# PolarisRisingWar/rgb-experiment

Hardware: AMD Instinct MI355X
Metric: aggregated edges/sec (full-graph GCN d=128, reference epoch = train fwd+bwd+Adam + 2 eval fwd) (higher is better)
Workload: dtype f32

## Files before the change

include/rgbx_hip.h:

```cpp
#ifndef RGBX_HIP_H
#define RGBX_HIP_H

#include <stddef.h>
#include <stdint.h>

#ifdef __cplusplus
extern "C" {
#endif

#define RGBX_VERSION 501

#define RGBX_OK 0
#define RGBX_E_ARG (-1)
#define RGBX_E_RANGE (-2)
#define RGBX_E_ALIGN (-3)
#define RGBX_E_WS (-4)
#define RGBX_E_SHAPE (-5)

typedef void* rgbx_stream_t;

enum {
  RGBX_LOOPS_KEEP = 0,
  RGBX_LOOPS_ADD_REMAINING = 1,
  RGBX_LOOPS_REMOVE_ADD = 2
// ... 307 lines not shown
int rgbx_gatv2_bwd_src_f32(const int32_t* rowptr_t, const int32_t* col_t, const int32_t* t2f, const float* xl,
                           int64_t ldl, const float* xr, int64_t ldr, const float* att, const float* nodeq,
                           const float* gout, int64_t ldg, float* g_xl, int64_t ldgl, int64_t N, int H, int C,
                           float slope, const uint32_t* seed, float p_drop, const rgbx_row_split_t* split,
                           rgbx_stream_t stream);

int rgbx_gatv2_draws_u8(const uint32_t* seed, int64_t nnz, int H, float p_drop, uint8_t* keep, rgbx_stream_t stream);


int rgbx_gemm_tn_workspace_bytes(int64_t K, int64_t M, int64_t N, size_t* bytes);

int rgbx_gemm_tn_f32(const float* A, int64_t lda, const float* B, int64_t ldb, float* C, int64_t ldc,
                     float* a_colsum, int64_t K, int64_t M, int64_t N, float alpha, void* workspace,
                     size_t workspace_bytes, rgbx_stream_t stream);


int rgbx_bn_scratch_doubles(int64_t N, int64_t d, int64_t* count);

int rgbx_bn_stats_f32(const float* x, int64_t ldx, int64_t N, int64_t d, double* sums, double* scratch,
                      int64_t scratch_doubles, rgbx_stream_t stream);

int rgbx_bn_finalize_f32(const double* packed, const float* weight, const float* bias, float eps, float momentum,
                         float* running_mean, float* running_var, float* mean, float* rstd, float* scale,
                         float* shift, int64_t d, rgbx_stream_t stream);

int rgbx_fold_bn_linear_f32(const float* W, int64_t ldw, const float* Wr, int64_t ldwr, const float* bias,
                            const float* bias2, const float* gamma, const float* beta, const float* running_mean,
                            const float* running_var, float eps, float* wt, float* wrt, float* b_out, int64_t Nout,
                            int64_t K, rgbx_stream_t stream);

// ... 92 lines not shown
```

rgb_experiment_amd/_lib.py:

```python
import ctypes
import os

import torch

_HERE = os.path.dirname(os.path.abspath(__file__))
LIB_PATH = os.path.join(_HERE, "csrc", "librgbx_hip.so")

_P = ctypes.c_void_p
_I64 = ctypes.c_int64
_I = ctypes.c_int
_F = ctypes.c_float

class RowSplit(ctypes.Structure):
    _fields_ = [("threshold", ctypes.c_int32), ("n_chunks", ctypes.c_int32), ("n_long", ctypes.c_int32),
                ("chunk_begin", ctypes.c_void_p), ("chunk_end", ctypes.c_void_p), ("chunk_row", ctypes.c_void_p),
                ("long_row", ctypes.c_void_p),
                ("long_chunk_ptr", ctypes.c_void_p), ("partial", ctypes.c_void_p)]


class MultiOut(ctypes.Structure):
    _fields_ = [(f, t) for name in ("sum", "mean", "var", "std", "max", "argmax", "min", "argmin")
                for f, t in ((name, ctypes.c_void_p), ("ld_" + name, ctypes.c_int64))]


# ... 83 lines not shown
                                  _P, _P],
    "rgbx_supergat_sample_negatives": [_P, _I64, _I64, _P, _I64, _I, _P, _P, _P],
    "rgbx_supergat_neg_loss_fwd_f32": [_P, _I64, _P, _P, _I64, _I, _I, _P, _I64, _P, _P],
    "rgbx_supergat_neg_loss_bwd_f32": [_P, _I64, _P, _P, _I64, _I, _I, _P, _P, _I64, _P],
    "rgbx_supergat_draws_u8": [_P, _I64, _I, _F, _F, _P, _P, _P],
    "rgbx_gatv2_supported": [_I, _I],
    "rgbx_gatv2_fwd_f32": [_P, _P, _P, _I64, _P, _I64, _P, _P, _P, _I64, _P, _P, _I64, _I, _I, _F, _P, _F, _P, _P],
    "rgbx_gatv2_att_partial_floats": [_I64, _I, _I, _P, ctypes.POINTER(ctypes.c_int64)],
    "rgbx_gatv2_bwd_dst_f32": [_P, _P, _P, _I64, _P, _I64, _P, _P, _P, _P, _I64, _P, _P, _I64, _P, _P, _I64, _P, _P, _I64,
                               _I64, _I, _I, _F, _P, _F, _P, _P],
    "rgbx_gatv2_bwd_src_f32": [_P, _P, _P, _P, _I64, _P, _I64, _P, _P, _P, _I64, _P, _I64, _I64, _I, _I, _F, _P, _F, _P,
                               _P],
    "rgbx_gatv2_draws_u8": [_P, _I64, _I, _F, _P, _P],
    "rgbx_gemm_tn_workspace_bytes": [_I64, _I64, _I64, ctypes.POINTER(ctypes.c_size_t)],
    "rgbx_gemm_tn_f32": [_P, _I64, _P, _I64, _P, _I64, _P, _I64, _I64, _I64, _F, _P, ctypes.c_size_t, _P],
    "rgbx_bn_scratch_doubles": [_I64, _I64, ctypes.POINTER(ctypes.c_int64)],
    "rgbx_bn_stats_f32": [_P, _I64, _I64, _I64, _P, _P, _I64, _P],
    "rgbx_bn_finalize_f32": [_P, _P, _P, _F, _F, _P, _P, _P, _P, _P, _P, _I64, _P],
    "rgbx_fold_bn_linear_f32": [_P, _I64, _P, _I64, _P, _P, _P, _P, _P, _P, _F, _P, _P, _P, _I64, _I64, _P],
    "rgbx_bn_bwd_finalize_f32": [_P, _P, _P, _P, _P, _P, _P, _P, _P, _P, _I64, _P],
    "rgbx_affine_cols_f32": [_P, _I64, _P, _P, _P, _I64, _I64, _I64, _P],
    "rgbx_bn_bwd_reduce_f32": [_P, _I64, _P, _I64, _P, _P, _I64, _I64, _P, _P, _I64, _P],
    "rgbx_bn_bwd_apply_f32": [_P, _I64, _P, _I64, _P, _P, _P, _P, _P, _P, _I64, _I64, _I64, _P],
    "rgbx_masked_nll_scratch_doubles": [_I64, _I, ctypes.POINTER(ctypes.c_int64)],
    "rgbx_masked_nll_fwd_f32": [_P, _I64, _P, _P, _I64, _I64, _P, _P, _I64, _I, _P],
    "rgbx_masked_ce_fwd_f32": [_P, _I64, _P, _P, _I64, _I64, _P, _P, _I64, _P],
    "rgbx_masked_ce_fwd_blocked_f32": [_P, _I64, _I64, _P, _P, _P, _I64, _I64, _P, _P, _I64, _P],
    "rgbx_masked_ce_bwd_f32": [_P, _I64, _P, _P, _I64, _I64, _P, _P, _I64, _P],
    "rgbx_masked_nll_bwd_f32": [_P, _P, _I64, _I64, _P, _P, _I64, _P],
    "rgbx_coalesce_workspace_bytes": [_I64, _I64, _I, ctypes.POINTER(ctypes.c_size_t)],
# ... 38 lines not shown
    if _lib is not None:
        return _lib
    if not os.path.exists(LIB_PATH):
        raise RuntimeError(
            f"rgb_experiment_amd: {LIB_PATH} is not built — run `python -c 'import __graft_entry__ as g; "
            "g.build()'` (or `make -C rgb_experiment_amd/csrc`). There is no CPU fallback.")
    _lib = bind(LIB_PATH)
    return _lib


def use(lib):
    global _lib
    _lib = lib


def check(rc, what):
    if rc != 0:
        msg = load().rgbx_last_error_string().decode(errors="replace")
        kind = "argument error" if rc < 0 else "hipError"
        raise RuntimeError(f"{what} failed ({kind} {rc}): {msg}")


def require_device(*tensors):
    for t in tensors:
        if t is not None and not t.is_cuda:
            raise RuntimeError(
                "rgb_experiment_amd: the message-passing path runs in HIP kernels on an MI355X device; "
                f"got a tensor on '{t.device}'. There is no CPU fallback (oracle/ is test-only).")


# ... 16 lines not shown
```

rgb_experiment_amd/csrc/bn.hip:

```cpp
#include "rgbx_common.h"

namespace rgbx {
namespace {

constexpr int kMaxBlocks = 1024;

struct ColMap {
  int cv;
  int rg;
};

__host__ __device__ inline ColMap col_map(int d, int vec) {
  int cv = (d + vec - 1) / vec;
  if (cv > 256) cv = 256;
  ColMap m{cv, 256 / cv};
  return m;
}

template <int VEC, bool BWD>
__global__ void __launch_bounds__(256)
col_reduce_kernel(const float* __restrict__ a, int64_t lda, const float* __restrict__ b, int64_t ldb,
                  const float* __restrict__ mean, const float* __restrict__ rstd, int64_t N, int d,
                  double* __restrict__ part) {
  extern __shared__ double sh[];
// ... 109 lines not shown
  const int per_row = (d + VEC - 1) / VEC;
  const int64_t total = N * per_row;
  for (int64_t idx = (int64_t)blockIdx.x * blockDim.x + threadIdx.x; idx < total;
       idx += (int64_t)gridDim.x * blockDim.x) {
    const int64_t r = idx / per_row;
    const int c = (int)(idx % per_row) * VEC;
    float g[VEC], v[VEC], mu[VEC], rs[VEC], a[VEC], b[VEC], k[VEC];
    load_vec<VEC>(g, gy + r * ldg + c);
    load_vec<VEC>(v, x + r * ldx + c);
    load_vec<VEC>(mu, mean + c);
    load_vec<VEC>(rs, rstd + c);
    load_vec<VEC>(a, ca + c);
    load_vec<VEC>(b, cb + c);
    load_vec<VEC>(k, ck + c);
#pragma unroll
    for (int i = 0; i < VEC; ++i) g[i] = (g[i] - a[i] - (v[i] - mu[i]) * rs[i] * b[i]) * k[i];
    store_vec<VEC>(gx + r * ldgx + c, g);
  }
}

int reduce_grid(int64_t N, int d, int vec) {
  const ColMap M = col_map(d, vec);
  int64_t b = cdiv(N, (int64_t)M.rg * 16);
  if (b > kMaxBlocks) b = kMaxBlocks;
  return (int)(b < 1 ? 1 : b);
}

bool vec4_ok(int64_t d, std::initializer_list<const void*> ptrs, std::initializer_list<int64_t> lds) {
  bool ok = d % 4 == 0;
  for (const void* p : ptrs) ok = ok && aligned16(p);
  for (int64_t ld : lds) ok = ok && ld % 4 == 0;
// ... 218 lines not shown
```

rgb_experiment_amd/csrc/gemm.hip:

```cpp
#include "rgbx_common.h"

namespace rgbx {
namespace {

constexpr int BM = 128, BN = 128, KT = 32;
using f32x16 = __attribute__((ext_vector_type(16))) float;

template <int W>
__device__ __forceinline__ void stage_tile(float* __restrict__ lds, const float* __restrict__ src,
                                           int64_t ld, int64_t k0, int64_t k_end, int c0, int ncols) {
  const int tid = threadIdx.x;
#pragma unroll 4
  for (int p = 0; p < KT * W / 256; ++p) {
    const int idx = p * 256 + tid;
    const int r = idx / W, c = idx % W;
    const int64_t k = k0 + r;
    lds[r * W + c] = (k < k_end && c0 + c < ncols) ? src[k * ld + c0 + c] : 0.f;
  }
}

template <int W>
__device__ __forceinline__ void fetch_tile(float4 (&regs)[KT * (W / 4) / 256], const float* __restrict__ src, int64_t ld,
                                           int64_t k0, int64_t k_end, int c0, int ncols) {
#pragma unroll
// ... 4 lines not shown
    regs[p] = make_float4(0.f, 0.f, 0.f, 0.f);
    if (k < k_end && c0 + c < ncols) regs[p] = *reinterpret_cast<const float4*>(src + k * ld + c0 + c);
  }
}

template <int W>
__device__ __forceinline__ void put_tile(float* __restrict__ lds, const float4 (&regs)[KT * (W / 4) / 256]) {
#pragma unroll
  for (int p = 0; p < KT * (W / 4) / 256; ++p) {
    const int idx = p * 256 + threadIdx.x;
    const int r = idx / (W / 4), c = (idx % (W / 4)) * 4;
    *reinterpret_cast<float4*>(lds + r * W + c) = regs[p];
  }
}

template <bool VEC4, int MT>
__global__ void __launch_bounds__(256)
gemm_tn_partial_kernel(const float* __restrict__ A, int64_t lda, const float* __restrict__ B, int64_t ldb,
                       float* __restrict__ part, float* __restrict__ colpart, int64_t K, int M, int N,
                       int64_t slab) {
  constexpr int MI = MT / 64;
  __shared__ float lds[KT * (MT + 128)];
  float* la = lds;
  float* lb = lds + KT * MT;
  const int split = blockIdx.x;
  const int m0 = blockIdx.y * MT, n0 = blockIdx.z * BN;
  const int64_t k_begin = (int64_t)split * slab;
  const int64_t k_end = k_begin + slab < K ? k_begin + slab : K;
  const int wave = threadIdx.x >> 6, lane = threadIdx.x & 63;
  const int wm = (wave >> 1) * (MT / 2), wn = (wave & 1) * 64;
  const int kr = lane >> 5, cc = lane & 31;

  f32x16 acc[MI][2];
#pragma unroll
  for (int i = 0; i < MI; ++i)
#pragma unroll
    for (int j = 0; j < 2; ++j)
#pragma unroll
      for (int r = 0; r < 16; ++r) acc[i][j][r] = 0.f;
// ... 7 lines not shown
    }
#pragma unroll 4
    for (int kk = 0; kk < KT; kk += 2) {
      float a[MI];
#pragma unroll
      for (int i = 0; i < MI; ++i) a[i] = la[(kk + kr) * MT + wm + i * 32 + cc];
      const float b0 = lb[(kk + kr) * 128 + wn + cc];
      const float b1 = lb[(kk + kr) * 128 + wn + 32 + cc];
#pragma unroll
      for (int i = 0; i < MI; ++i) {
        acc[i][0] = __builtin_amdgcn_mfma_f32_32x32x2f32(a[i], b0, acc[i][0], 0, 0, 0);
        acc[i][1] = __builtin_amdgcn_mfma_f32_32x32x2f32(a[i], b1, acc[i][1], 0, 0, 0);
      }
    }
  };
  if constexpr (VEC4) {
    float4 ra[KT * (MT / 4) / 256], rb[KT * 32 / 256];
    fetch_tile<MT>(ra, A, lda, k_begin, k_end, m0, M);
    fetch_tile<128>(rb, B, ldb, k_begin, k_end, n0, N);
    for (int64_t k0 = k_begin; k0 < k_end; k0 += KT) {
      __syncthreads();
      put_tile<MT>(la, ra);
      put_tile<128>(lb, rb);
      __syncthreads();
      if (k0 + KT < k_end) {
        fetch_tile<MT>(ra, A, lda, k0 + KT, k_end, m0, M);
        fetch_tile<128>(rb, B, ldb, k0 + KT, k_end, n0, N);
      }
      consume();
    }
  } else {
// ... 53 lines not shown
  return (int)s;
}

}
}

using namespace rgbx;

extern "C" int rgbx_gemm_tn_workspace_bytes(int64_t K, int64_t M, int64_t N, size_t* bytes) {
  if (!bytes || K < 0 || M < 0 || N < 0) return fail(RGBX_E_ARG, "gemm_tn_workspace_bytes: bad argument");
  if (M >= INT32_MAX || N >= INT32_MAX) return fail(RGBX_E_RANGE, "gemm_tn: M or N exceeds int32");
  *bytes = (size_t)choose_splits(K, (int)M, (int)N) * ((size_t)M * (size_t)N + (size_t)M) * sizeof(float);
  return RGBX_OK;
}

extern "C" int rgbx_gemm_tn_f32(const float* A, int64_t lda, const float* B, int64_t ldb, float* C,
                                int64_t ldc, float* a_colsum, int64_t K, int64_t M, int64_t N, float alpha,
                                void* workspace, size_t workspace_bytes, rgbx_stream_t stream) {
  if (K < 0 || M < 0 || N < 0) return fail(RGBX_E_ARG, "gemm_tn: negative size");
  if (M == 0 || N == 0) return RGBX_OK;
  if (!C || (K > 0 && (!A || !B))) return fail(RGBX_E_ARG, "gemm_tn: null pointer");
  if (M >= INT32_MAX || N >= INT32_MAX) return fail(RGBX_E_RANGE, "gemm_tn: M or N exceeds int32");
  if (lda < M || ldb < N || ldc < N) return fail(RGBX_E_ARG, "gemm_tn: leading dimension too small");
  size_t need = 0;
  if (int rc = rgbx_gemm_tn_workspace_bytes(K, M, N, &need)) return rc;
  if (!workspace || workspace_bytes < need)
    return fail(RGBX_E_WS, "gemm_tn: workspace %zu < %zu bytes", workspace_bytes, need);
  hipStream_t s = (hipStream_t)stream;
  const int S = choose_splits(K, (int)M, (int)N);
  const int64_t slab = cdiv(cdiv(K > 0 ? K : 1, S), KT) * KT;
  float* part = static_cast<float*>(workspace);
  float* colpart = a_colsum ? part + (size_t)S * M * N : nullptr;
  const int mt = tile_rows((int)M);
  dim3 grid(S, (unsigned)cdiv(M, mt), (unsigned)cdiv(N, BN));
  const bool v4 = aligned16(A) && aligned16(B) && lda % 4 == 0 && ldb % 4 == 0;
#define RGBX_GEMM_TN(V4, MT) \
  gemm_tn_partial_kernel<V4, MT><<<grid, 256, 0, s>>>(A, lda, B, ldb, part, colpart, K, (int)M, (int)N, slab)
  if (v4) { if (mt == 64) RGBX_GEMM_TN(true, 64); else RGBX_GEMM_TN(true, 128); }
  else { if (mt == 64) RGBX_GEMM_TN(false, 64); else RGBX_GEMM_TN(false, 128); }
#undef RGBX_GEMM_TN
  RGBX_CHECK_LAUNCH("gemm_tn_partial_kernel");
  const int64_t MN = M * N;
  int64_t rb = cdiv(MN, 32);
  if (rb > kMaxGrid) rb = kMaxGrid;
  gemm_tn_reduce_kernel<<<(int)rb, 256, 0, s>>>(part, S, MN, C, (int)N, ldc, alpha);
  RGBX_CHECK_LAUNCH("gemm_tn_reduce_kernel");
  if (a_colsum) {
    gemm_tn_reduce_kernel<<<(int)cdiv(M, 32), 256, 0, s>>>(colpart, S, M, a_colsum, (int)M, M, 1.0f);
    RGBX_CHECK_LAUNCH("gemm_tn_reduce_kernel");
  }
  return RGBX_OK;
}
```

rgb_experiment_amd/csrc/rgbx_common.h:

```cpp
#pragma once
#include <cstring>
#include <hip/hip_runtime.h>

#include <algorithm>
#include <cstdarg>
#include <cstdint>
#include <cstdio>
#include <initializer_list>

#include "../../include/rgbx_hip.h"

namespace rgbx {

constexpr int kWave = 64;

char* err_buf();

inline int fail(int code, const char* fmt, ...) {
  va_list ap;
  va_start(ap, fmt);
  vsnprintf(err_buf(), 256, fmt, ap);
  va_end(ap);
  return code;
}
// ... 31 lines not shown
  if constexpr (VEC == 4) { v[0] = t.x; v[1] = t.y; v[2] = t.z; v[3] = t.w; }
  else if constexpr (VEC == 2) { v[0] = t.x; v[1] = t.y; }
  else { v[0] = t; }
}

template <int VEC>
__device__ __forceinline__ void store_vec(float* p, const float (&v)[VEC]) {
  using V = typename VecT<VEC>::type;
  V t;
  if constexpr (VEC == 4) { t.x = v[0]; t.y = v[1]; t.z = v[2]; t.w = v[3]; }
  else if constexpr (VEC == 2) { t.x = v[0]; t.y = v[1]; }
  else { t = v[0]; }
  *reinterpret_cast<V*>(p) = t;
}

constexpr int kMaxGrid = 256 * 8 * 4;

}
```

rgb_experiment_amd/models/_stack.py:

```python
import torch
import torch.nn as nn
import torch.nn.functional as F

from ..nn import BatchNorm1d


class ModelOutput(dict):

    _LAZY = ("out", "x")

    def __init__(self, logits):
        super().__init__(emb=logits)

    def _log_probs(self):
        out = F.log_softmax(dict.__getitem__(self, "emb"), dim=1)
        dict.__setitem__(self, "out", out)
        dict.__setitem__(self, "x", out)
        return out

    def __missing__(self, key):
        if key in self._LAZY:
            return self._log_probs()
        raise KeyError(key)

# ... 95 lines not shown
                res = conv.forward_folded(x, edge_index, folded[i], ce=ce if i == last else None, **ew)
                if res is not None:
                    x = res
                    continue
            extra = dict(ew)
            if (bn is not None and bn.training and torch.is_grad_enabled() and getattr(conv, "emits_colsums", False)
                    and hasattr(bn, "begin_training_step")):
                extra["want_colsums"] = True
            if (i == last and ce is not None and getattr(conv, "accepts_ce", False)
                    and (not isinstance(ce[1], (tuple, list)) or getattr(conv, "accepts_ce_pair", False))):
                extra["ce"] = ce
            if pending is not None:
                sums = getattr(x, ops.COLSUMS, None)
                after = getattr(conv, "forward_after_bn", None)
                if after is not None:
                    x, pending = after(x, edge_index, pending, colsums=sums, **extra), bn
                    continue
                x, pending = (pending(x, colsums=sums) if sums is not None else pending(x)), None
            affine = None
            if bn is not None and getattr(conv, "folds_post_affine", False) and not torch.is_grad_enabled():
                fold = getattr(bn, "eval_affine", None)
                affine = fold() if fold is not None else None
            if affine is not None:
                x = conv(x, edge_index, post_affine=affine, **ew)
            else:
                x, pending = conv(x, edge_index, **extra), bn
        if ce is not None and not isinstance(x, tuple):
            x = ops.ce_from_logits(x, ce[0], ce[1])
        return x


# ... 152 lines not shown
```

rgb_experiment_amd/nn/batchnorm.py:

```python
import ctypes

import torch
import torch.nn as nn

from .. import _lib


def _scratch(n, d, device):
    cnt = ctypes.c_int64(0)
    _lib.check(_lib.load().rgbx_bn_scratch_doubles(n, d, ctypes.byref(cnt)), "rgbx_bn_scratch_doubles")
    return torch.empty(cnt.value, dtype=torch.float64, device=device), cnt.value


def column_sums(x):
    if not x.is_cuda:
        xd = x.double()
        return torch.stack([xd.sum(0), (xd * xd).sum(0)])
    px, ldx = _lib.mat(x, "x")
    n, d = x.shape
    sums = torch.empty((2, d), dtype=torch.float64, device=x.device)
    scratch, cnt = _scratch(n, d, x.device)
    _lib.check(_lib.load().rgbx_bn_stats_f32(px, ldx, n, d, _lib.ptr(sums), _lib.ptr(scratch), cnt, _lib.stream_ptr()),
               "rgbx_bn_stats_f32")
    return sums
# ... 75 lines not shown
    else:
        mean64 = packed[:d] / n
        var64 = (packed[d:2 * d] / n - mean64 * mean64).clamp_(min=0.0)
        mean, var = mean64.float(), var64.float()
        rstd = torch.rsqrt(var + eps)
        scale = weight.detach() * rstd
        shift = bias.detach() - mean * scale
        if running is not None:
            rm, rv, mom = running
            unbiased = var * (n / (n - 1).clamp(min=1)).float()
            rm.mul_(1 - mom).add_(mean, alpha=mom)
            rv.mul_(1 - mom).add_(unbiased, alpha=mom)
    return mean, rstd, scale, shift, n


def train_backward(gy, x, weight, mean, rstd, n, reduce, grads_out=None, sums=None):
    gy = gy if gy.stride(-1) == 1 else gy.contiguous()
    d = x.size(1)
    if sums is None:
        local = bwd_sums(gy, x, mean, rstd)
        glob = reduce(local.reshape(-1).clone())
    else:
        local, glob = sums
    if gy.is_cuda:
        ca, cb, ck = (torch.empty(d, dtype=torch.float32, device=gy.device) for _ in range(3))
        gw, gb = grads_out if grads_out is not None else (torch.empty(d, dtype=torch.float32, device=gy.device)
                                                          for _ in range(2))
        _lib.check(_lib.load().rgbx_bn_bwd_finalize_f32(
            _lib.ptr(glob), _lib.ptr(local), _lib.ptr(n), _lib.ptr(weight.detach().contiguous()), _lib.ptr(rstd),
            _lib.ptr(ca), _lib.ptr(cb), _lib.ptr(ck), _lib.ptr(gw), _lib.ptr(gb), d, _lib.stream_ptr()),
            "rgbx_bn_bwd_finalize_f32")
    else:
        glob = glob.reshape(2, -1)
        ca = (glob[0] / n).float().contiguous()
        cb = (glob[1] / n).float().contiguous()
        ck = (weight * rstd).contiguous()
        gw, gb = local[1].float(), local[0].float()
        if grads_out is not None:
            grads_out[0].copy_(gw)
            grads_out[1].copy_(gb)
            gw, gb = grads_out
    return bwd_apply(gy, x, mean, rstd, ca, cb, ck), gw, gb


class _AffineCols(torch.autograd.Function):

    @staticmethod
    def forward(ctx, x, scale, shift):
        x = x if x.stride(-1) == 1 else x.contiguous()
        ctx.save_for_backward(x, scale)
        return affine_cols(x, scale.detach().contiguous(), shift.detach().contiguous())

    @staticmethod
    def backward(ctx, gy):
        x, scale = ctx.saved_tensors
        gy = gy if gy.stride(-1) == 1 else gy.contiguous()
# ... 47 lines not shown
```

rgb_experiment_amd/ops.py:

```python
import ctypes

import torch

from . import _lib

_EVENT_SINK = None


def set_event_sink(sink):
    global _EVENT_SINK
    _EVENT_SINK = sink


class Kind(str):
    variant = None


class _Timed:
    def __init__(self, kind, variant=None):
        if variant is not None and _EVENT_SINK is not None:
            kind = Kind(kind)
            kind.variant = variant
        self.kind = kind

# ... 848 lines not shown
    def forward(ctx, z, weight, bias, root_weight, x_root, want_colsums):
        out, _, cs = fused_layer(z, weight_t(weight), bias=None if bias is None else bias.detach(),
                                 x_root=x_root if root_weight is not None else None,
                                 wt_root=None if root_weight is None else weight_t(root_weight),
                                 want_colsums=want_colsums, kind="cached_aggregate_linear_fwd")
        ctx.save_for_backward(z, x_root if root_weight is not None else None)
        ctx.has_bias = bias is not None
        if want_colsums:
            ctx.mark_non_differentiable(cs)
            return out, cs
        return out

    @staticmethod
    def backward(ctx, gy, _g_cs=None):
        z, x_root = ctx.saved_tensors
        gy = gy.contiguous()
        gw = gb = gwr = None
        want_b = ctx.has_bias and ctx.needs_input_grad[2]
        if ctx.needs_input_grad[1]:
            if want_b:
                gw, gb = gemm_tn(gy, z, colsum=True)
            else:
                gw = gemm_tn(gy, z)
        elif want_b:
            gb = gy.sum(0)
        if x_root is not None and ctx.needs_input_grad[3]:
            gwr = gemm_tn(gy, x_root)
        return None, gw, gb, gwr, None, None


def aggregate_linear_ok(in_channels, out_channels, root=False):
    return bool(_lib.load().rgbx_spmm_linear_supported(in_channels, out_channels, int(root)))


def aggregate_linear(z, weight, bias=None, root_weight=None, x_root=None, want_colsums=False):
    return _tag_colsums(_AggregateLinear.apply(z, weight, bias, root_weight, x_root, want_colsums), want_colsums)


def fold_bn_linear(weight, bias=None, bias2=None, root_weight=None, bn=None):
    _lib.require_device(weight, bias, bias2, root_weight)
    W = weight.detach()
    W = W if W.stride(-1) == 1 else W.contiguous()
    n_out, K = W.shape
    Wr = None
    if root_weight is not None:
        Wr = root_weight.detach()
        Wr = Wr if Wr.stride(-1) == 1 else Wr.contiguous()
    wt = torch.empty((K, n_out), dtype=torch.float32, device=W.device)
    wrt = torch.empty_like(wt) if Wr is not None else None
    has_b = bias is not None or bias2 is not None or bn is not None
    b_out = torch.empty(n_out, dtype=torch.float32, device=W.device) if has_b else None
# ... 24 lines not shown
                              need_z, xr if root_weight is not None else None,
                              None if root_weight is None else weight_t(root_weight),
                              kind=f"{getattr(graph, 'event_prefix', '')}{kind}_linear_fwd", want_colsums=want_colsums)
        out, z = res[0], res[1]
        ctx.save_for_backward(z, weight, root_weight, xr if root_weight is not None else None)
        ctx.graph, ctx.kind, ctx.has_bias = graph, kind, bias is not None
        if want_colsums:
            ctx.mark_non_differentiable(res[2])
            return out, res[2]
        return out

    @staticmethod
    def backward(ctx, gy, _g_colsums=None):
        z, weight, root_weight, x = ctx.saved_tensors
        g, kind = ctx.graph, ctx.kind
        gy = gy.contiguous()
        gx = gw = gb = gwr = None
        want_b = ctx.has_bias and ctx.needs_input_grad[4]
        if ctx.needs_input_grad[3]:
            if want_b:
                gw, gb = gemm_tn(gy, z, colsum=True)
            else:
                gw = gemm_tn(gy, z)
        elif want_b:
            gb = gy.sum(0)
        if root_weight is not None and ctx.needs_input_grad[6]:
            gwr = gemm_tn(gy, x)
        if ctx.needs_input_grad[0]:
            gx = _propagate_linear_input_grad(g, kind, gy, weight, root_weight)
        return gx, None, None, gw, gb, None, gwr, None, None


def _propagate_linear_input_grad(g, kind, gy, weight, root_weight, ce_sel=None):
# ... 6 lines not shown
                               x_root=gy if root_weight is not None else None,
                               wt_root=None if root_weight is None else root_weight.detach().contiguous(),
                               col_sel=None if ce_sel is None else selected_cols(*ce_sel), kind=f"{prefix}{kind}_linear_bwd")
        return gx
    gz = gy @ weight
    gr = gy @ root_weight if root_weight is not None else None
    if gr is None:
        return spmm_raw(csr, wt, None, gz, kind=f"{prefix}{kind}_bwd")
    return spmm_raw(csr, wt, None, gz, y=gr, a=1.0, b=1.0, out=gr, kind=f"{prefix}{kind}_bwd")


class _BNPropagateLinear(torch.autograd.Function):

    @staticmethod
    def forward(ctx, x, bn_weight, bn_bias, graph, kind, weight, bias, root_weight, eps, reduce, running, need_z,
                colsums=None, want_colsums=False):
        from .nn import batchnorm as B
        x = x.contiguous()
        mean, rstd, scale, shift, n = B.train_statistics(x, bn_weight, bn_bias, eps, reduce, running, colsums)
        w, rs = (graph.w, None) if kind == "gcn" else (None, graph.inv_deg)
        res = spmm_linear_raw(graph.fwd, w, rs, x, weight_t(weight), None if bias is None else bias.detach(), need_z,
                              x if root_weight is not None else None,
                              None if root_weight is None else weight_t(root_weight), kind=f"{kind}_linear_fwd",
                              pre=(scale, shift, graph.rowsum(kind)), want_colsums=want_colsums)
        out, z = res[0], res[1]
        ctx.save_for_backward(x, bn_weight, mean, rstd, n, z, weight, root_weight, scale, shift)
        ctx.graph, ctx.kind, ctx.has_bias, ctx.reduce = graph, kind, bias is not None, reduce
        if want_colsums:
            ctx.mark_non_differentiable(res[2])
            return out, res[2]
        return out

# ... 1 lines not shown
    def backward(ctx, gy, _g_colsums=None):
        from .nn import batchnorm as B
        x, bn_weight, mean, rstd, n, z, weight, root_weight, scale, shift = ctx.saved_tensors
        g, kind = ctx.graph, ctx.kind
        gy = gy.contiguous()
        gw = gb = gwr = None
        if ctx.needs_input_grad[5]:
            gw, gcol = gemm_tn(gy, z, colsum=True)
            gb = gcol if ctx.has_bias and ctx.needs_input_grad[6] else None
        else:
            gcol = gy.sum(0)
            gb = gcol if ctx.has_bias and ctx.needs_input_grad[6] else None
        if root_weight is not None and ctx.needs_input_grad[7]:
            gwr = gemm_tn(gy, x) * scale + gcol[:, None] * shift
        g_h = _propagate_linear_input_grad(g, kind, gy, weight, root_weight)
        gx, g_bnw, g_bnb = B.train_backward(g_h, x, bn_weight, mean, rstd, n, ctx.reduce)
        return gx, g_bnw, g_bnb, None, None, gw, gb, gwr, None, None, None, None, None, None


_SCALE_CACHE = {}


def mask_scale(y, mask, C):
    key = (y.data_ptr(), y._version, y.numel(), None if mask is None else (mask.data_ptr(), mask._version), int(C))
    hit = _SCALE_CACHE.get(key)
    if hit is None:
        sel = (y >= 0) & (y < C)
        if mask is not None:
            sel = sel & mask.bool()
        hit = (_MadeOn((1.0 / sel.sum().double()).float().reshape(1)), y, mask)
        _SCALE_CACHE[key] = hit
        while len(_SCALE_CACHE) > 32:
# ... 73 lines not shown


def fused_ce_ok(graph, in_channels, out_channels, root, x, y):
    return (not _is_dist(graph) and out_channels <= 128 and y is not None and y.is_cuda and y.dtype == torch.int64
            and fused_linear_ok(graph, in_channels, out_channels, root=root, x=x))


class _PropagateLinearCE(torch.autograd.Function):

    @staticmethod
    def forward(ctx, x, graph, kind, weight, bias, root_weight, y, mask, want_grad, bn_weight, bn_bias, bn_args):
        from .nn import batchnorm as B
        x = x.contiguous()
        pre = None
        if bn_weight is not None:
            eps, reduce, running, colsums = bn_args
            mean, rstd, scale, shift, n = B.train_statistics(x, bn_weight, bn_bias, eps, reduce, running, colsums)
            pre = (scale, shift, graph.rowsum(kind))
        w, rs = (graph.w, None) if kind == "gcn" else (None, graph.inv_deg)
        grad_scale = mask_scale(y, mask, weight.size(0)) if want_grad else None
        dlogits, z, stats = spmm_linear_raw(
            graph.fwd, w, rs, x, weight_t(weight), None if bias is None else bias.detach(),
            want_grad and weight.requires_grad, x if root_weight is not None else None,
            None if root_weight is None else weight_t(root_weight), kind=f"{kind}_linear_fwd", pre=pre,
            ce=(y, mask, grad_scale), select_rows=True)
        ctx.graph, ctx.kind, ctx.has_bias, ctx.has_bn = graph, kind, bias is not None, bn_weight is not None
        ctx.ce_sel = (y, mask, weight.size(0)) if want_grad else None
        if want_grad:
            if ctx.has_bn:
                ctx.save_for_backward(dlogits, z, weight, root_weight, x, bn_weight, mean, rstd, n, scale, shift)
                ctx.reduce = bn_args[1]
# ... 25 lines not shown
                gcol = gcol if gcol is not None else gy.sum(0)
                gwr = gemm_tn(gy, x) * scale + gcol[:, None] * shift
            else:
                gwr = gemm_tn(gy, x)
        need_h = ctx.needs_input_grad[0] or (ctx.has_bn and (ctx.needs_input_grad[9] or ctx.needs_input_grad[10]))
        items = [(k, t) for k, t in (("gw", gw), ("gb", gb), ("gwr", gwr)) if t is not None]
        if need_h:
            items.append(("w", weight.detach()))
            if root_weight is not None:
                items.append(("wr", root_weight.detach()))
        sc = dict(zip((k for k, _ in items), torch._foreach_mul([t for _, t in items], g))) if items else {}
        gw, gb, gwr = sc.get("gw"), sc.get("gb"), sc.get("gwr")
        if need_h:
            g_h = _propagate_linear_input_grad(graph, kind, gy, sc["w"], sc.get("wr"), ce_sel=ctx.ce_sel)
            if ctx.has_bn:
                gx, g_bnw, g_bnb = B.train_backward(g_h, x, bn_weight, mean, rstd, n, ctx.reduce)
            else:
                gx = g_h
        return gx, None, None, gw, gb, gwr, None, None, None, g_bnw, g_bnb, None


def propagate_linear_ce(x, graph, kind, weight, bias, root_weight, y, mask, bn=None, colsums=None):
    want_grad = not isinstance(mask, (tuple, list)) and torch.is_grad_enabled() and any(
        t is not None and t.requires_grad
        for t in (weight, x, bias, root_weight) + ((bn.weight, bn.bias) if bn is not None else ()))
    if bn is not None:
        bn_args = (bn.eps, bn._reduce, bn.begin_training_step(), colsums)
        return _PropagateLinearCE.apply(x, graph, kind, weight, bias, root_weight, y, mask, want_grad, bn.weight, bn.bias,
                                        bn_args)
    return _PropagateLinearCE.apply(x, graph, kind, weight, bias, root_weight, y, mask, want_grad, None, None, None)


def bn_propagate_linear(x, bn, graph, kind, weight, bias=None, root_weight=None, colsums=None, want_colsums=False):
    need_z = weight.requires_grad
    return _tag_colsums(_BNPropagateLinear.apply(x, bn.weight, bn.bias, graph, kind, weight, bias, root_weight, bn.eps,
                                                 bn._reduce, bn.begin_training_step(), need_z, colsums, want_colsums),
                        want_colsums)


COLSUMS = "_rgbx_colsums"


def _tag_colsums(res, want_colsums):
    if not want_colsums:
        return res
    out, colsums = res
    setattr(out, COLSUMS, colsums)
    return out


def propagate_linear(x, graph, kind, weight, bias=None, root_weight=None, want_colsums=False):
    if _is_dist(graph):
        return graph.propagate_linear(x, kind, weight, bias, root_weight)
    need_z = torch.is_grad_enabled() and weight.requires_grad
    return _tag_colsums(_PropagateLinear.apply(x, graph, kind, weight, bias, need_z, root_weight, None, want_colsums),
                        want_colsums)


def appnp_raw(csr, w, h, K, alpha, kind="appnp"):
    _lib.require_device(h)
    h = h.contiguous()
    ph, ldh = _lib.mat(h, "h")
    out = torch.empty_like(h)
    tmp = torch.empty_like(h) if K > 1 else None
    po, ldo = _lib.mat(out, "out")
    split, _scratch = csr.split_arg(h.size(1), h.device)
    with _Timed(kind):
        _lib.check(
            _lib.load().rgbx_appnp_f32(_lib.ptr(csr.rowptr), _lib.ptr(csr.col), _lib.ptr(w), ph, ldh, po,
                                       _lib.ptr(tmp), ldo, csr.N, h.size(1), int(K), float(alpha),
                                       None if split is None else ctypes.byref(split), _lib.stream_ptr()),
# ... 1083 lines not shown
    if out is None:
        out = torch.empty((M, N), dtype=torch.float32, device=a.device)
    elif tuple(out.shape) != (M, N) or not out.is_contiguous() or out.dtype != torch.float32:
        raise RuntimeError(f"gemm_tn: out must be a contiguous float32 [{M}, {N}] tensor")
    sums = None
    if colsum:
        sums = sums_out if sums_out is not None else torch.empty(M, dtype=torch.float32, device=a.device)
        if tuple(sums.shape) != (M,) or not sums.is_contiguous() or sums.dtype != torch.float32:
            raise RuntimeError(f"gemm_tn: sums_out must be a contiguous float32 [{M}] tensor")
    with _Timed("gemm_tn", f"{M}x{N}" if _EVENT_SINK is not None else None):
        _lib.check(lib.rgbx_gemm_tn_f32(pa, lda, pb, ldb, _lib.ptr(out), N, _lib.ptr(sums), K, M, N, float(alpha),
                                        _lib.ptr(ws), ws.numel(), _lib.stream_ptr()), "rgbx_gemm_tn_f32")
    return (out, sums) if colsum else out


class _Linear(torch.autograd.Function):

    @staticmethod
    def forward(ctx, x, weight, bias):
        ctx.save_for_backward(x, weight)
        ctx.has_bias = bias is not None
        if _EVENT_SINK is None or not x.is_cuda:
            return torch.nn.functional.linear(x, weight, bias)
        with _Timed("linear_fwd", f"{weight.size(1)}->{weight.size(0)}"):
            return torch.nn.functional.linear(x, weight, bias)

    @staticmethod
    def backward(ctx, gy):
        x, weight = ctx.saved_tensors
        gy = gy.contiguous()
# ... 272 lines not shown
```

Baseline: 16.70 billion.

## Fuse BatchNorm input-grad apply into the downstream weight-gradient GEMM

Instead of writing the full BatchNorm input gradient and then reading it back for the next layer's weight-gradient GEMM, the BN backward returns a lazy placeholder carrying g, x and the per-column coefficients. A new GEMM-TN variant forms the BN-corrected gradient while loading A tiles, reading g and x plus five per-column vectors staged in LDS. This removes one N×d write and one read plus a kernel launch when the consumer is the sole reader and no input gradient is needed. In exchange, the GEMM reads two input streams per A tile, uses more registers and LDS, and depends on tagging logic to decide when the hand-off is safe.

```diff
diff --git a/include/rgbx_hip.h b/include/rgbx_hip.h
--- a/include/rgbx_hip.h
+++ b/include/rgbx_hip.h
@@ -345,6 +345,11 @@
                      float* a_colsum, int64_t K, int64_t M, int64_t N, float alpha, void* workspace,
                      size_t workspace_bytes, rgbx_stream_t stream);
 
+int rgbx_gemm_tn_bnbwd_f32(const float* g, int64_t ldg, const float* x, int64_t ldx, const float* mean,
+                           const float* rstd, const float* ca, const float* cb, const float* ck, const float* B,
+                           int64_t ldb, float* C, int64_t ldc, float* a_colsum, int64_t K, int64_t M, int64_t N,
+                           float alpha, void* workspace, size_t workspace_bytes, rgbx_stream_t stream);
+
 
 int rgbx_bn_scratch_doubles(int64_t N, int64_t d, int64_t* count);
 
diff --git a/rgb_experiment_amd/_lib.py b/rgb_experiment_amd/_lib.py
--- a/rgb_experiment_amd/_lib.py
+++ b/rgb_experiment_amd/_lib.py
@@ -121,6 +121,8 @@
     "rgbx_gatv2_draws_u8": [_P, _I64, _I, _F, _P, _P],
     "rgbx_gemm_tn_workspace_bytes": [_I64, _I64, _I64, ctypes.POINTER(ctypes.c_size_t)],
     "rgbx_gemm_tn_f32": [_P, _I64, _P, _I64, _P, _I64, _P, _I64, _I64, _I64, _F, _P, ctypes.c_size_t, _P],
+    "rgbx_gemm_tn_bnbwd_f32": [_P, _I64, _P, _I64, _P, _P, _P, _P, _P, _P, _I64, _P, _I64, _P, _I64, _I64, _I64, _F, _P,
+                               ctypes.c_size_t, _P],
     "rgbx_bn_scratch_doubles": [_I64, _I64, ctypes.POINTER(ctypes.c_int64)],
     "rgbx_bn_stats_f32": [_P, _I64, _I64, _I64, _P, _P, _I64, _P],
     "rgbx_bn_finalize_f32": [_P, _P, _P, _F, _F, _P, _P, _P, _P, _P, _P, _I64, _P],
@@ -189,6 +191,9 @@
     _lib = lib
 
 
+E_ALIGN, E_SHAPE = -3, -5
+
+
 def check(rc, what):
     if rc != 0:
         msg = load().rgbx_last_error_string().decode(errors="replace")
diff --git a/rgb_experiment_amd/csrc/bn.hip b/rgb_experiment_amd/csrc/bn.hip
--- a/rgb_experiment_amd/csrc/bn.hip
+++ b/rgb_experiment_amd/csrc/bn.hip
@@ -147,7 +147,7 @@
     load_vec<VEC>(b, cb + c);
     load_vec<VEC>(k, ck + c);
 #pragma unroll
-    for (int i = 0; i < VEC; ++i) g[i] = (g[i] - a[i] - (v[i] - mu[i]) * rs[i] * b[i]) * k[i];
+    for (int i = 0; i < VEC; ++i) g[i] = bn_bwd_elem(g[i], v[i], mu[i], rs[i], a[i], b[i], k[i]);
     store_vec<VEC>(gx + r * ldgx + c, g);
   }
 }
diff --git a/rgb_experiment_amd/csrc/gemm.hip b/rgb_experiment_amd/csrc/gemm.hip
--- a/rgb_experiment_amd/csrc/gemm.hip
+++ b/rgb_experiment_amd/csrc/gemm.hip
@@ -42,15 +42,43 @@
   }
 }
 
-template <bool VEC4, int MT>
-__global__ void __launch_bounds__(256)
+struct BnBwdOperand {
+  const float* x;
+  int64_t ldx;
+  const float *mean, *rstd, *ca, *cb, *ck;
+};
+
+template <int W>
+__device__ __forceinline__ void put_tile_bnbwd(float* __restrict__ lds, float4 (&rg)[KT * (W / 4) / 256],
+                                               const float4 (&rx)[KT * (W / 4) / 256], const float* __restrict__ lc,
+                                               int64_t k0, int64_t k_end, int c0, int ncols) {
+  const int c = (threadIdx.x % (W / 4)) * 4;
+  const bool col_ok = c0 + c < ncols;
+#pragma unroll
+  for (int j = 0; j < 4; ++j) {
+    const float mu = lc[c + j], rs = lc[W + c + j], a = lc[2 * W + c + j], b = lc[3 * W + c + j], k = lc[4 * W + c + j];
+#pragma unroll
+    for (int p = 0; p < KT * (W / 4) / 256; ++p) {
+      float& g = j == 0 ? rg[p].x : j == 1 ? rg[p].y : j == 2 ? rg[p].z : rg[p].w;
+      const float x = j == 0 ? rx[p].x : j == 1 ? rx[p].y : j == 2 ? rx[p].z : rx[p].w;
+      const int r = (p * 256 + threadIdx.x) / (W / 4);
+      g = (col_ok && k0 + r < k_end) ? bn_bwd_elem(g, x, mu, rs, a, b, k) : 0.f;
+    }
+  }
+  put_tile<W>(lds, rg);
+}
+
+template <bool VEC4, int MT, bool BNBWD = false>
+__global__ void __launch_bounds__(256) __attribute__((amdgpu_waves_per_eu(BNBWD ? 3 : 1)))
 gemm_tn_partial_kernel(const float* __restrict__ A, int64_t lda, const float* __restrict__ B, int64_t ldb,
                        float* __restrict__ part, float* __restrict__ colpart, int64_t K, int M, int N,
-                       int64_t slab) {
+                       int64_t slab, BnBwdOperand bn) {
+  static_assert(!BNBWD || VEC4, "the A operand is formed on load on the 16-byte path only");
   constexpr int MI = MT / 64;
-  __shared__ float lds[KT * (MT + 128)];
+  __shared__ float lds[KT * (MT + 128) + (BNBWD ? 5 * MT : 0)];
   float* la = lds;
   float* lb = lds + KT * MT;
+  float* lc = lds + KT * (MT + 128);
   const int split = blockIdx.x;
   const int m0 = blockIdx.y * MT, n0 = blockIdx.z * BN;
   const int64_t k_begin = (int64_t)split * slab;
@@ -88,7 +116,32 @@
       }
     }
   };
-  if constexpr (VEC4) {
+  if constexpr (BNBWD) {
+    float4 ra[KT * (MT / 4) / 256], rx[KT * (MT / 4) / 256], rb[KT * 32 / 256];
+    fetch_tile<MT>(ra, A, lda, k_begin, k_end, m0, M);
+    fetch_tile<MT>(rx, bn.x, bn.ldx, k_begin, k_end, m0, M);
+    fetch_tile<128>(rb, B, ldb, k_begin, k_end, n0, N);
+    for (int i = threadIdx.x; i < MT; i += 256) {
+      const bool in = m0 + i < M;
+      lc[i] = in ? bn.mean[m0 + i] : 0.f;
+      lc[MT + i] = in ? bn.rstd[m0 + i] : 0.f;
+      lc[2 * MT + i] = in ? bn.ca[m0 + i] : 0.f;
+      lc[3 * MT + i] = in ? bn.cb[m0 + i] : 0.f;
+      lc[4 * MT + i] = in ? bn.ck[m0 + i] : 0.f;
+    }
+    for (int64_t k0 = k_begin; k0 < k_end; k0 += KT) {
+      __syncthreads();
+      put_tile_bnbwd<MT>(la, ra, rx, lc, k0, k_end, m0, M);
+      put_tile<128>(lb, rb);
+      __syncthreads();
+      if (k0 + KT < k_end) {
+        fetch_tile<MT>(ra, A, lda, k0 + KT, k_end, m0, M);
+        fetch_tile<MT>(rx, bn.x, bn.ldx, k0 + KT, k_end, m0, M);
+        fetch_tile<128>(rb, B, ldb, k0 + KT, k_end, n0, N);
+      }
+      consume();
+    }
+  } else if constexpr (VEC4) {
     float4 ra[KT * (MT / 4) / 256], rb[KT * 32 / 256];
     fetch_tile<MT>(ra, A, lda, k_begin, k_end, m0, M);
     fetch_tile<128>(rb, B, ldb, k_begin, k_end, n0, N);
@@ -172,14 +225,9 @@
   return RGBX_OK;
 }
 
-extern "C" int rgbx_gemm_tn_f32(const float* A, int64_t lda, const float* B, int64_t ldb, float* C,
-                                int64_t ldc, float* a_colsum, int64_t K, int64_t M, int64_t N, float alpha,
-                                void* workspace, size_t workspace_bytes, rgbx_stream_t stream) {
-  if (K < 0 || M < 0 || N < 0) return fail(RGBX_E_ARG, "gemm_tn: negative size");
-  if (M == 0 || N == 0) return RGBX_OK;
-  if (!C || (K > 0 && (!A || !B))) return fail(RGBX_E_ARG, "gemm_tn: null pointer");
-  if (M >= INT32_MAX || N >= INT32_MAX) return fail(RGBX_E_RANGE, "gemm_tn: M or N exceeds int32");
-  if (lda < M || ldb < N || ldc < N) return fail(RGBX_E_ARG, "gemm_tn: leading dimension too small");
+static int run_gemm_tn(const float* A, int64_t lda, const float* B, int64_t ldb, float* C, int64_t ldc, float* a_colsum,
+                       int64_t K, int64_t M, int64_t N, float alpha, void* workspace, size_t workspace_bytes,
+                       rgbx_stream_t stream, const BnBwdOperand* bn) {
   size_t need = 0;
   if (int rc = rgbx_gemm_tn_workspace_bytes(K, M, N, &need)) return rc;
   if (!workspace || workspace_bytes < need)
@@ -193,10 +241,15 @@
   dim3 grid(S, (unsigned)cdiv(M, mt), (unsigned)cdiv(N, BN));
   const bool v4 = aligned16(A) && aligned16(B) && lda % 4 == 0 && ldb % 4 == 0;
 #define RGBX_GEMM_TN(V4, MT) \
-  gemm_tn_partial_kernel<V4, MT><<<grid, 256, 0, s>>>(A, lda, B, ldb, part, colpart, K, (int)M, (int)N, slab)
-  if (v4) { if (mt == 64) RGBX_GEMM_TN(true, 64); else RGBX_GEMM_TN(true, 128); }
+  gemm_tn_partial_kernel<V4, MT><<<grid, 256, 0, s>>>(A, lda, B, ldb, part, colpart, K, (int)M, (int)N, slab, \
+                                                      BnBwdOperand{})
+#define RGBX_GEMM_TN_BNBWD(MT) \
+  gemm_tn_partial_kernel<true, MT, true><<<grid, 256, 0, s>>>(A, lda, B, ldb, part, colpart, K, (int)M, (int)N, slab, *bn)
+  if (bn) { if (mt == 64) RGBX_GEMM_TN_BNBWD(64); else RGBX_GEMM_TN_BNBWD(128); }
+  else if (v4) { if (mt == 64) RGBX_GEMM_TN(true, 64); else RGBX_GEMM_TN(true, 128); }
   else { if (mt == 64) RGBX_GEMM_TN(false, 64); else RGBX_GEMM_TN(false, 128); }
 #undef RGBX_GEMM_TN
+#undef RGBX_GEMM_TN_BNBWD
   RGBX_CHECK_LAUNCH("gemm_tn_partial_kernel");
   const int64_t MN = M * N;
   int64_t rb = cdiv(MN, 32);
@@ -209,3 +262,32 @@
   }
   return RGBX_OK;
 }
+
+extern "C" int rgbx_gemm_tn_f32(const float* A, int64_t lda, const float* B, int64_t ldb, float* C,
+                                int64_t ldc, float* a_colsum, int64_t K, int64_t M, int64_t N, float alpha,
+                                void* workspace, size_t workspace_bytes, rgbx_stream_t stream) {
+  if (K < 0 || M < 0 || N < 0) return fail(RGBX_E_ARG, "gemm_tn: negative size");
+  if (M == 0 || N == 0) return RGBX_OK;
+  if (!C || (K > 0 && (!A || !B))) return fail(RGBX_E_ARG, "gemm_tn: null pointer");
+  if (M >= INT32_MAX || N >= INT32_MAX) return fail(RGBX_E_RANGE, "gemm_tn: M or N exceeds int32");
+  if (lda < M || ldb < N || ldc < N) return fail(RGBX_E_ARG, "gemm_tn: leading dimension too small");
+  return run_gemm_tn(A, lda, B, ldb, C, ldc, a_colsum, K, M, N, alpha, workspace, workspace_bytes, stream, nullptr);
+}
+
+extern "C" int rgbx_gemm_tn_bnbwd_f32(const float* g, int64_t ldg, const float* x, int64_t ldx, const float* mean,
+                                      const float* rstd, const float* ca, const float* cb, const float* ck,
+                                      const float* B, int64_t ldb, float* C, int64_t ldc, float* a_colsum, int64_t K,
+                                      int64_t M, int64_t N, float alpha, void* workspace, size_t workspace_bytes,
+                                      rgbx_stream_t stream) {
+  if (K < 0 || M < 0 || N < 0) return fail(RGBX_E_ARG, "gemm_tn_bnbwd: negative size");
+  if (M == 0 || N == 0) return RGBX_OK;
+  if (!C || !mean || !rstd || !ca || !cb || !ck || (K > 0 && (!g || !x || !B)))
+    return fail(RGBX_E_ARG, "gemm_tn_bnbwd: null pointer");
+  if (M >= INT32_MAX || N >= INT32_MAX) return fail(RGBX_E_RANGE, "gemm_tn_bnbwd: M or N exceeds int32");
+  if (ldg < M || ldx < M || ldb < N || ldc < N) return fail(RGBX_E_ARG, "gemm_tn_bnbwd: leading dimension too small");
+  if (M % 4 != 0) return fail(RGBX_E_SHAPE, "gemm_tn_bnbwd: M = %lld is not a multiple of 4", (long long)M);
+  if (!(aligned16(g) && aligned16(x) && aligned16(B) && ldg % 4 == 0 && ldx % 4 == 0 && ldb % 4 == 0))
+    return fail(RGBX_E_ALIGN, "gemm_tn_bnbwd: g, x and B need 16-byte aligned rows");
+  const BnBwdOperand bn{x, ldx, mean, rstd, ca, cb, ck};
+  return run_gemm_tn(g, ldg, B, ldb, C, ldc, a_colsum, K, M, N, alpha, workspace, workspace_bytes, stream, &bn);
+}
diff --git a/rgb_experiment_amd/csrc/rgbx_common.h b/rgb_experiment_amd/csrc/rgbx_common.h
--- a/rgb_experiment_amd/csrc/rgbx_common.h
+++ b/rgb_experiment_amd/csrc/rgbx_common.h
@@ -69,6 +69,11 @@
   *reinterpret_cast<V*>(p) = t;
 }
 
+__device__ __forceinline__ float bn_bwd_elem(float g, float x, float mean, float rstd, float ca, float cb, float ck) {
+  const float xhat = (x - mean) * rstd;
+  return fmaf(-xhat, cb, g - ca) * ck;
+}
+
 constexpr int kMaxGrid = 256 * 8 * 4;
 
 }
diff --git a/rgb_experiment_amd/models/_stack.py b/rgb_experiment_amd/models/_stack.py
--- a/rgb_experiment_amd/models/_stack.py
+++ b/rgb_experiment_amd/models/_stack.py
@@ -133,7 +133,7 @@
                 sums = getattr(x, ops.COLSUMS, None)
                 after = getattr(conv, "forward_after_bn", None)
                 if after is not None:
-                    x, pending = after(x, edge_index, pending, colsums=sums, **extra), bn
+                    x, pending = after(ops.sole_reader(x), edge_index, pending, colsums=sums, **extra), bn
                     continue
                 x, pending = (pending(x, colsums=sums) if sums is not None else pending(x)), None
             affine = None
diff --git a/rgb_experiment_amd/nn/batchnorm.py b/rgb_experiment_amd/nn/batchnorm.py
--- a/rgb_experiment_amd/nn/batchnorm.py
+++ b/rgb_experiment_amd/nn/batchnorm.py
@@ -113,7 +113,7 @@
     return mean, rstd, scale, shift, n
 
 
-def train_backward(gy, x, weight, mean, rstd, n, reduce, grads_out=None, sums=None):
+def train_backward(gy, x, weight, mean, rstd, n, reduce, grads_out=None, sums=None, defer_apply=False):
     gy = gy if gy.stride(-1) == 1 else gy.contiguous()
     d = x.size(1)
     if sums is None:
@@ -139,6 +139,9 @@
             grads_out[0].copy_(gw)
             grads_out[1].copy_(gb)
             gw, gb = grads_out
+    if defer_apply and gy.is_cuda:
+        from .. import ops
+        return ops.BNInputGrad(gy, x, mean, rstd, ca, cb, ck).placeholder(), gw, gb
     return bwd_apply(gy, x, mean, rstd, ca, cb, ck), gw, gb
 
 
diff --git a/rgb_experiment_amd/ops.py b/rgb_experiment_amd/ops.py
--- a/rgb_experiment_amd/ops.py
+++ b/rgb_experiment_amd/ops.py
@@ -886,9 +886,15 @@
     @staticmethod
     def backward(ctx, gy, _g_cs=None):
         z, x_root = ctx.saved_tensors
-        gy = gy.contiguous()
         gw = gb = gwr = None
         want_b = ctx.has_bias and ctx.needs_input_grad[2]
+        pend = take_bn_input_grad(gy)
+        if pend is not None:
+            if x_root is None and ctx.needs_input_grad[1]:
+                gw, gcol = gemm_tn_bnbwd(pend, z)
+                return None, gw, gcol if want_b else None, None, None, None
+            gy = pend.materialize()
+        gy = gy.contiguous()
         if ctx.needs_input_grad[1]:
             if want_b:
                 gw, gb = gemm_tn(gy, z, colsum=True)
@@ -906,7 +912,8 @@
 
 
 def aggregate_linear(z, weight, bias=None, root_weight=None, x_root=None, want_colsums=False):
-    return _tag_colsums(_AggregateLinear.apply(z, weight, bias, root_weight, x_root, want_colsums), want_colsums)
+    out = _tag_colsums(_AggregateLinear.apply(z, weight, bias, root_weight, x_root, want_colsums), want_colsums)
+    return _tag_takes_bn_input_grad(out, z, weight, root_weight)
 
 
 def fold_bn_linear(weight, bias=None, bias2=None, root_weight=None, bn=None):
@@ -961,9 +968,15 @@
     def backward(ctx, gy, _g_colsums=None):
         z, weight, root_weight, x = ctx.saved_tensors
         g, kind = ctx.graph, ctx.kind
-        gy = gy.contiguous()
         gx = gw = gb = gwr = None
         want_b = ctx.has_bias and ctx.needs_input_grad[4]
+        pend = take_bn_input_grad(gy)
+        if pend is not None:
+            if root_weight is None and ctx.needs_input_grad[3] and not ctx.needs_input_grad[0]:
+                gw, gcol = gemm_tn_bnbwd(pend, z)
+                return None, None, None, gw, gcol if want_b else None, None, None, None, None
+            gy = pend.materialize()
+        gy = gy.contiguous()
         if ctx.needs_input_grad[3]:
             if want_b:
                 gw, gb = gemm_tn(gy, z, colsum=True)
@@ -1000,8 +1013,9 @@
 
     @staticmethod
     def forward(ctx, x, bn_weight, bn_bias, graph, kind, weight, bias, root_weight, eps, reduce, running, need_z,
-                colsums=None, want_colsums=False):
+                colsums=None, want_colsums=False, defer_gx=False):
         from .nn import batchnorm as B
+        ctx.defer_gx = defer_gx
         x = x.contiguous()
         mean, rstd, scale, shift, n = B.train_statistics(x, bn_weight, bn_bias, eps, reduce, running, colsums)
         w, rs = (graph.w, None) if kind == "gcn" else (None, graph.inv_deg)
@@ -1033,8 +1047,8 @@
         if root_weight is not None and ctx.needs_input_grad[7]:
             gwr = gemm_tn(gy, x) * scale + gcol[:, None] * shift
         g_h = _propagate_linear_input_grad(g, kind, gy, weight, root_weight)
-        gx, g_bnw, g_bnb = B.train_backward(g_h, x, bn_weight, mean, rstd, n, ctx.reduce)
-        return gx, g_bnw, g_bnb, None, None, gw, gb, gwr, None, None, None, None, None, None
+        gx, g_bnw, g_bnb = B.train_backward(g_h, x, bn_weight, mean, rstd, n, ctx.reduce, defer_apply=ctx.defer_gx)
+        return gx, g_bnw, g_bnb, None, None, gw, gb, gwr, None, None, None, None, None, None, None
 
 
 _SCALE_CACHE = {}
@@ -1138,7 +1152,7 @@
         x = x.contiguous()
         pre = None
         if bn_weight is not None:
-            eps, reduce, running, colsums = bn_args
+            eps, reduce, running, colsums, ctx.defer_gx = bn_args
             mean, rstd, scale, shift, n = B.train_statistics(x, bn_weight, bn_bias, eps, reduce, running, colsums)
             pre = (scale, shift, graph.rowsum(kind))
         w, rs = (graph.w, None) if kind == "gcn" else (None, graph.inv_deg)
@@ -1194,7 +1208,8 @@
         if need_h:
             g_h = _propagate_linear_input_grad(graph, kind, gy, sc["w"], sc.get("wr"), ce_sel=ctx.ce_sel)
             if ctx.has_bn:
-                gx, g_bnw, g_bnb = B.train_backward(g_h, x, bn_weight, mean, rstd, n, ctx.reduce)
+                gx, g_bnw, g_bnb = B.train_backward(g_h, x, bn_weight, mean, rstd, n, ctx.reduce,
+                                                    defer_apply=ctx.defer_gx)
             else:
                 gx = g_h
         return gx, None, None, gw, gb, gwr, None, None, None, g_bnw, g_bnb, None
@@ -1205,7 +1220,7 @@
         t is not None and t.requires_grad
         for t in (weight, x, bias, root_weight) + ((bn.weight, bn.bias) if bn is not None else ()))
     if bn is not None:
-        bn_args = (bn.eps, bn._reduce, bn.begin_training_step(), colsums)
+        bn_args = (bn.eps, bn._reduce, bn.begin_training_step(), colsums, want_grad and hands_over_bn_input_grad(x))
         return _PropagateLinearCE.apply(x, graph, kind, weight, bias, root_weight, y, mask, want_grad, bn.weight, bn.bias,
                                         bn_args)
     return _PropagateLinearCE.apply(x, graph, kind, weight, bias, root_weight, y, mask, want_grad, None, None, None)
@@ -1214,7 +1229,8 @@
 def bn_propagate_linear(x, bn, graph, kind, weight, bias=None, root_weight=None, colsums=None, want_colsums=False):
     need_z = weight.requires_grad
     return _tag_colsums(_BNPropagateLinear.apply(x, bn.weight, bn.bias, graph, kind, weight, bias, root_weight, bn.eps,
-                                                 bn._reduce, bn.begin_training_step(), need_z, colsums, want_colsums),
+                                                 bn._reduce, bn.begin_training_step(), need_z, colsums, want_colsums,
+                                                 hands_over_bn_input_grad(x)),
                         want_colsums)
 
 
@@ -1229,12 +1245,57 @@
     return out
 
 
+
+FUSE_BN_BWD_DW = True
+TAKES_BN_INPUT_GRAD = "_rgbx_takes_bn_input_grad"
+SOLE_READER = "_rgbx_sole_reader"
+BN_INPUT_GRAD = "_rgbx_bn_input_grad"
+
+
+class BNInputGrad:
+    __slots__ = ("g", "x", "mean", "rstd", "ca", "cb", "ck")
+
+    def __init__(self, g, x, mean, rstd, ca, cb, ck):
+        self.g, self.x, self.mean, self.rstd, self.ca, self.cb, self.ck = g, x, mean, rstd, ca, cb, ck
+
+    def materialize(self):
+        from .nn import batchnorm as B
+        return B.bwd_apply(self.g, self.x, self.mean, self.rstd, self.ca, self.cb, self.ck)
+
+    def placeholder(self):
+        t = torch.empty(1, dtype=self.g.dtype, device=self.g.device).expand(self.x.size(0), self.x.size(1))
+        setattr(t, BN_INPUT_GRAD, self)
+        return t
+
+
+def take_bn_input_grad(gy):
+    return getattr(gy, BN_INPUT_GRAD, None)
+
+
+def _tag_takes_bn_input_grad(out, x, weight, root_weight):
+    if (FUSE_BN_BWD_DW and torch.is_grad_enabled() and out.is_cuda and not x.requires_grad and root_weight is None
+            and weight.requires_grad):
+        setattr(out, TAKES_BN_INPUT_GRAD, True)
+    return out
+
+
+def sole_reader(x):
+    if getattr(x, TAKES_BN_INPUT_GRAD, False):
+        setattr(x, SOLE_READER, True)
+    return x
+
+
+def hands_over_bn_input_grad(x):
+    return bool(FUSE_BN_BWD_DW and getattr(x, TAKES_BN_INPUT_GRAD, False) and getattr(x, SOLE_READER, False))
+
+
 def propagate_linear(x, graph, kind, weight, bias=None, root_weight=None, want_colsums=False):
     if _is_dist(graph):
         return graph.propagate_linear(x, kind, weight, bias, root_weight)
     need_z = torch.is_grad_enabled() and weight.requires_grad
-    return _tag_colsums(_PropagateLinear.apply(x, graph, kind, weight, bias, need_z, root_weight, None, want_colsums),
-                        want_colsums)
+    out = _tag_colsums(_PropagateLinear.apply(x, graph, kind, weight, bias, need_z, root_weight, None, want_colsums),
+                       want_colsums)
+    return _tag_takes_bn_input_grad(out, x, weight, root_weight) if need_z else out
 
 
 def appnp_raw(csr, w, h, K, alpha, kind="appnp"):
@@ -2348,6 +2409,37 @@
     return (out, sums) if colsum else out
 
 
+def gemm_tn_bnbwd(pend, b, out=None, sums_out=None):
+    g, x = pend.g, pend.x
+    _lib.require_device(g, x, b)
+    if g.stride(-1) != 1 or x.stride(-1) != 1:
+        return gemm_tn(pend.materialize(), b, colsum=True, out=out, sums_out=sums_out)
+    b = b if b.stride(-1) == 1 and _rows_padded_readable(b) else b.contiguous()
+    if g.size(0) >= 4096:
+        b = _aligned_rows(b)
+    pg, ldg = _lib.mat(g, "g")
+    px, ldx = _lib.mat(x, "x")
+    pb, ldb = _lib.mat(b, "b")
+    K, M, N = g.size(0), g.size(1), b.size(1)
+    lib = _lib.load()
+    nbytes = ctypes.c_size_t(0)
+    _lib.check(lib.rgbx_gemm_tn_workspace_bytes(K, M, N, ctypes.byref(nbytes)), "rgbx_gemm_tn_workspace_bytes")
+    ws = torch.empty(max(nbytes.value, 1), dtype=torch.uint8, device=g.device)
+    dw = out if out is not None else torch.empty((M, N), dtype=torch.float32, device=g.device)
+    sums = sums_out if sums_out is not None else torch.empty(M, dtype=torch.float32, device=g.device)
+    if (tuple(dw.shape) != (M, N) or not dw.is_contiguous() or dw.dtype != torch.float32
+            or tuple(sums.shape) != (M,) or not sums.is_contiguous() or sums.dtype != torch.float32):
+        raise RuntimeError(f"gemm_tn_bnbwd: out / sums_out must be contiguous float32 [{M}, {N}] / [{M}] tensors")
+    with _Timed("gemm_tn", f"bnbwd {M}x{N}" if _EVENT_SINK is not None else None):
+        rc = lib.rgbx_gemm_tn_bnbwd_f32(pg, ldg, px, ldx, _lib.ptr(pend.mean), _lib.ptr(pend.rstd), _lib.ptr(pend.ca),
+                                        _lib.ptr(pend.cb), _lib.ptr(pend.ck), pb, ldb, _lib.ptr(dw), N, _lib.ptr(sums), K,
+                                        M, N, 1.0, _lib.ptr(ws), ws.numel(), _lib.stream_ptr())
+    if rc in (_lib.E_ALIGN, _lib.E_SHAPE):
+        return gemm_tn(pend.materialize(), b, colsum=True, out=out, sums_out=sums_out)
+    _lib.check(rc, "rgbx_gemm_tn_bnbwd_f32")
+    return dw, sums
+
+
 class _Linear(torch.autograd.Function):
 
     @staticmethod
```

Result: no change. 16.93 billion (median of 3 runs) (+1.4%).
